# smpurkis/PyTorch-Face-Detection-from-Scratch

Hardware: AMD Instinct MI355X
Metric: train imgs/sec (PoolResnet 480^2, bs=256 per GPU) (higher is better)
Workload: dtype f32 (3x3 convs: bf16x3 split MFMA, fp32 accumulate)

## Files before the change

include/fdet.h:

```cpp
#ifndef FDET_H
#define FDET_H

#include <stddef.h>
#include <stdint.h>

#ifdef __cplusplus
extern "C" {
#endif

#define FDET_VERSION 100
#define FDET_OK 0
#define FDET_EINVAL (-1)
#define FDET_ELAUNCH (-2)
#define FDET_EWORKSPACE (-3)

int fdet_version(void);
const char* fdet_last_error(void);


int fdet_encode_targets(const float* boxes, const int32_t* box_offset, int B, int S,
                        float img_w, float img_h, float* out, void* stream);

int fdet_yolo_loss_fwd_bwd(const float* pred, const float* gt, int B, int S,
                           float* loss_per_image, float* loss_sum, float* grad_pred,
                           float grad_scale, void* stream);

int fdet_decode(const float* maps, int B, int S, float prob_threshold, float img_w, float img_h,
                float* scores, float* boxes, int32_t* counts, void* stream);

int fdet_nms(const float* boxes, const float* scores, const int32_t* counts, int B, int Kmax,
             double iou_threshold, int32_t* keep, int32_t* keep_counts, void* stream);

int fdet_reduce_bounding_boxes(const float* maps, int B, int S, float prob_threshold,
                               double iou_threshold, float img_w, float img_h,
                               float* out, int32_t* out_counts, void* stream);

int fdet_step_metrics(const float* gt, const int32_t* gt_counts, const float* pred,
                      const int32_t* pred_counts, int B, int Kmax, float* per_image,
                      float* totals, void* stream);

// ... 610 lines not shown
```

pytorch-face-detection-from-scratch_amd/_native.py:

```python
from __future__ import annotations

import ctypes
import os
import re
import subprocess
from typing import Optional

import torch

_HERE = os.path.dirname(os.path.abspath(__file__))
LIB_PATH = os.environ.get("FDET_LIB_PATH") or os.path.join(_HERE, "lib", "libfdet_hip.so")
HEADER_PATH = os.path.join(os.path.dirname(_HERE), "include", "fdet.h")


class FdetError(RuntimeError):
    pass


def build(verbose: bool = False) -> str:
    cmd = ["make", "-C", os.path.join(_HERE, "csrc"), "-j", str(min(8, os.cpu_count() or 1))]
    r = subprocess.run(cmd, capture_output=True, text=True)
    if verbose or r.returncode != 0:
        print(r.stdout[-4000:])
        print(r.stderr[-8000:])
    if r.returncode != 0:
        raise FdetError("building libfdet_hip.so failed (see compiler output above)")
    return LIB_PATH


_c = ctypes
_P, _I, _F, _D, _SZ, _U64, _U32 = _c.c_void_p, _c.c_int, _c.c_float, _c.c_double, _c.c_size_t, _c.c_uint64, _c.c_uint32

SIGNATURES = {
    "fdet_version": (_I, []),
    "fdet_last_error": (_c.c_char_p, []),
    "fdet_encode_targets": (_I, [_P, _P, _I, _I, _F, _F, _P, _P]),
    "fdet_yolo_loss_fwd_bwd": (_I, [_P, _P, _I, _I, _P, _P, _P, _F, _P]),
    "fdet_decode": (_I, [_P, _I, _I, _F, _F, _F, _P, _P, _P, _P]),
    "fdet_nms": (_I, [_P, _P, _P, _I, _I, _D, _P, _P, _P]),
    "fdet_reduce_bounding_boxes": (_I, [_P, _I, _I, _F, _D, _F, _F, _P, _P, _P]),
    "fdet_step_metrics": (_I, [_P, _P, _P, _P, _I, _I, _P, _P, _P]),
    "fdet_ssd_num_priors": (_I, [_P, _I]),
    "fdet_ssd_encode_targets": (_I, [_P, _P, _I, _P, _I, _F, _F, _P, _P]),
    "fdet_ssd_loss_ws_bytes": (_SZ, [_I]),
    "fdet_ssd_loss_fwd_bwd": (_I, [_P, _P, _I, _I, _I, _P, _P, _P, _P, _SZ, _P]),
    "fdet_ssd_loss_parts": (_I, [_P, _P, _I, _I, _I, _P, _P, _P, _P, _SZ, _P]),
    "fdet_ssd_loss_finish": (_I, [_P, _P, _P, _SZ, _P, _SZ, _P]),
    "fdet_ssd_reduce_bounding_boxes": (_I, [_P, _I, _P, _I, _I, _F, _D, _F, _F, _P, _P, _P]),
    "fdet_ssd_reduce_bounding_boxes_priors": (_I, [_P, _I, _P, _I, _I, _P, _F, _D, _F, _F, _P, _P, _P]),
    "fdet_ssd_head_pack_fwd": (_I, [_P, _I, _I, _I, _I, _I, _P, _P]),
    "fdet_ssd_head_pack_bwd": (_I, [_P, _P, _I, _I, _I, _I, _I, _P, _P]),
    "fdet_u8_to_f32_norm": (_I, [_P, _P, _SZ, _P]),
    "fdet_resize_bilinear_u8_norm": (_I, [_P, _P, _I, _I, _I, _I, _I, _I, _P]),
    "fdet_resize_bilinear_f32_norm": (_I, [_P, _P, _I, _I, _I, _I, _I, _I, _F, _P]),
    "fdet_adam_step": (_I, [_P, _P, _P, _P, _SZ, _I, _D, _D, _D, _D, _F, _P]),
    "fdet_pack_conv3x3_weights": (_I, [_P, _I, _I, _P, _P, _P]),
    "fdet_conv3x3_fwd": (_I, [_P, _P, _P, _P, _P, _P, _P, _I, _I, _I, _I, _I, _I, _F, _P]),
    "fdet_conv3x3_dgrad": (_I, [_P, _P, _P, _P, _P, _I, _I, _I, _I, _I, _F, _P]),
# ... 221 lines not shown
```

pytorch-face-detection-from-scratch_amd/csrc/fdet_conv3x3_x3.hip:

```cpp
#include "fdet_conv3x3_x3.h"
#include <algorithm>

namespace {

long long* g_probe_stamps = nullptr;
constexpr int PACK_MAXL = 32;
struct PackBatch { const float* w[PACK_MAXL]; bf16x8* fwd[PACK_MAXL]; bf16x8* bwd[PACK_MAXL]; };

__device__ __forceinline__ void pack3x3_x3(const float* __restrict__ w, int Cout, int Cin, int CoP, int CiP,
                                           bf16x8* __restrict__ fwd, bf16x8* __restrict__ bwd) {
  const int nf = (Cin / 16) * 9 * 2 * CoP, nb = (Cout / 16) * 9 * 2 * CiP;
  const int t = blockIdx.x * 256 + threadIdx.x;
  if (fwd && t < nf) {
    const int co = t % CoP, r = t / CoP;
    const int h = r & 1, r2 = r >> 1, tap = r2 % 9, c16 = r2 / 9;
    float f[8];
#pragma unroll
    for (int j = 0; j < 8; ++j) f[j] = (co < Cout) ? w[((size_t)co * Cin + c16 * 16 + 8 * h + j) * 9 + tap] : 0.f;
    bf16x8 hi, lo;
    split8(f, hi, lo);
    fwd[t] = hi;
    fwd[nf + t] = lo;
  }
  if (bwd && t < nb) {
    const int ci = t % CiP, r = t / CiP;
    const int h = r & 1, r2 = r >> 1, tap = r2 % 9, o16 = r2 / 9;
    float f[8];
#pragma unroll
    for (int j = 0; j < 8; ++j) f[j] = (ci < Cin) ? w[((size_t)(o16 * 16 + 8 * h + j) * Cin + ci) * 9 + (8 - tap)] : 0.f;
    bf16x8 hi, lo;
    split8(f, hi, lo);
    bwd[t] = hi;
    bwd[nb + t] = lo;
  }
}

__global__ void __launch_bounds__(256)
k_pack3x3_x3(const float* __restrict__ w, int Cout, int Cin, int CoP, int CiP, bf16x8* __restrict__ fwd,
             bf16x8* __restrict__ bwd) {
  pack3x3_x3(w, Cout, Cin, CoP, CiP, fwd, bwd);
}

__global__ void __launch_bounds__(256)
k_pack3x3_x3_batched(const PackBatch b, int Cout, int Cin, int CoP, int CiP) {
  pack3x3_x3(b.w[blockIdx.y], Cout, Cin, CoP, CiP, b.fwd[blockIdx.y], b.bwd[blockIdx.y]);
}

int run_x3(ConvArgs a, hipStream_t st) {
  static const char kernel_choice = [] { const char* e = getenv("FDET_CONV_KERNEL"); return e ? e[0] : '\0'; }();
  if (a.W <= 64 && kernel_choice != 'g') {
    static const int sb_al = [] { const char* e = getenv("FDET_SB_AL"); return e ? (e[0] == '1' ? 1 : 0) : -1; }();
    if (sb_al == 1 || (sb_al < 0 && a.W >= 33)) {
// ... 284 lines not shown
```

pytorch-face-detection-from-scratch_amd/csrc/fdet_head_fused.hip:

```cpp
#include "fdet_common.h"
#include <cfloat>

using namespace fdet;

typedef __bf16 hf_bf16x8 __attribute__((ext_vector_type(8)));
typedef float hf_f32x4 __attribute__((ext_vector_type(4)));

namespace {

constexpr int HF_T = 512;
constexpr int HF_F = 64;
constexpr int HF_K = 6;
constexpr int HF_KK = HF_K * HF_K;
constexpr int HF_XPT = 248;
constexpr int HF_XTP = 248;
constexpr int HF_DZOFF = (HF_K - 1) * 16 + (HF_K - 1);
constexpr int HF_DZP = 328;
constexpr int HF_DQ = 160;
constexpr int HF_OFF_XB = 0;
constexpr int HF_OFF_XT = HF_OFF_XB + 2 * 8 * HF_XPT * 16;
constexpr int HF_OFF_DZ = HF_OFF_XT + 2 * HF_F * HF_XTP * 2;
constexpr int HF_OFF_DZT = HF_OFF_DZ + 2 * HF_DZP * 16;
constexpr int HF_OFF_PART = HF_OFF_DZT + HF_K * 2 * 5 * HF_DQ * 2;
constexpr int HF_OFF_SC = HF_OFF_PART + 2 * 5 * 160 * 4;
// ... 327 lines not shown
      for (int i = tid; i < a.N; i += 256) s += __hip_atomic_load(a.lpi + i, __ATOMIC_RELAXED, __HIP_MEMORY_SCOPE_AGENT);
      red[tid] = s;
    }
    __syncthreads();
    for (int w = 128; w > 0; w >>= 1) {
      if (tid < w) red[tid] += red[tid + w];
      __syncthreads();
    }
    if (tid == 0) {
      a.lsum[0] = red[0] * 1.0f;
      *a.counter = 0u;
    }
  }
}

__global__ void __launch_bounds__(256)
k_head_fused_pack(const float* __restrict__ w, hf_bf16x8* __restrict__ wf, hf_bf16x8* __restrict__ wd) {
  const int t = blockIdx.x * 256 + threadIdx.x;
  const int nwf = HF_KK * 2 * 4 * 8, nwd = HF_KK * HF_F;
  if (t < nwf) {
    const int slot = t & 7, kgp = (t >> 3) & 3, c32 = (t >> 5) & 1, tap = t >> 6;
    float v[8];
#pragma unroll
    for (int j = 0; j < 8; ++j) v[j] = slot < 5 ? w[((size_t)slot * HF_F + 32 * c32 + 8 * kgp + j) * HF_KK + tap] : 0.f;
    hf_bf16x8 hi, lo;
    hf_split8(v, hi, lo);
    wf[t] = hi;
    wf[nwf + t] = lo;
  } else if (t < nwf + nwd) {
    const int u = t - nwf, c = u & 63, tap = u >> 6;
    float v[8];
#pragma unroll
    for (int j = 0; j < 8; ++j) v[j] = j < 5 ? w[((size_t)j * HF_F + c) * HF_KK + tap] : 0.f;
    hf_bf16x8 hi, lo;
    hf_split8(v, hi, lo);
    wd[u] = hi;
    wd[nwd + u] = lo;
  }
}

__global__ void __launch_bounds__(1024)
k_head_fused_reduce(const float* __restrict__ wsW, const float* __restrict__ wsb, int N, float* __restrict__ dW,
                    float* __restrict__ db) {
  __shared__ float part[1024];
  const int q = threadIdx.x & 63, ph = threadIdx.x >> 6;
  const int nS = HF_KK * 5 * HF_F;
  const int t = blockIdx.x * 64 + q;
  float s = 0.f;
  if (t < nS) {
    for (int n = ph; n < N; n += 16) s += wsW[(size_t)n * nS + t];
  } else if (t < nS + 5) {
    for (int n = ph; n < N; n += 16) s += wsb[(size_t)n * 8 + (t - nS)];
  }
  part[threadIdx.x] = s;
  __syncthreads();
  if (ph == 0) {
    float tot = 0.f;
#pragma unroll
    for (int p = 0; p < 16; ++p) tot += part[p * 64 + q];
    if (t < nS) {
      const int c = t & 63, r = t >> 6, o = r % 5, tap = r / 5;
      dW[((size_t)o * HF_F + c) * HF_KK + tap] = tot;
    } else if (t < nS + 5) {
      db[t - nS] = tot;
    }
  }
}

constexpr size_t hf_pack_units() { return (size_t)2 * HF_KK * 2 * 4 * 8 + (size_t)2 * HF_KK * HF_F; }

}

extern "C" int fdet_head_loss_fused_supported(int F, int H, int W, int k, int pad) {
  const int So = H - k + 1, Wo = W - k + 1;
  return F == HF_F && k == HF_K && pad == 0 && H >= k && W >= k && H <= 15 && W <= 15 && So <= 10 && 5 * So * Wo <= HF_T;
}
// ... 41 lines not shown
```

pytorch-face-detection-from-scratch_amd/csrc/fdet_stem_x3.hip:

```cpp
#include "fdet_common.h"
#include "fdet_ps.h"
#include "fdet_q8_common.h"
#include <algorithm>
#include <cstdlib>
#include <utility>

using namespace fdet;
typedef float f32x16 __attribute__((ext_vector_type(16)));
typedef float f32x4 __attribute__((ext_vector_type(4)));
typedef __bf16 bf16x8 __attribute__((ext_vector_type(8)));
typedef __bf16 bf16x4 __attribute__((ext_vector_type(4)));

namespace {

constexpr int KS = 10, ST = 8, PD = 2, CIN = 3;
constexpr int NROW = CIN * KS;
constexpr int RL = 8 * 64 + 16;
constexpr int RC = RL / 8;
constexpr int NSLOT = 15;

struct StemX3Args {
  const float* x; const float* w; const float* bias; float* y;
  int N, F, H, W, Ho, Wo, nrows;
  int ps_hp, ps_wp, ps_plane, ps_img;
  float q_inv;
};

__global__ void __launch_bounds__(256, 1)
k_stem_fwd_x3(const StemX3Args a) {
  extern __shared__ __attribute__((aligned(16))) char smem[];
  __bf16* Xh = reinterpret_cast<__bf16*>(smem);
  __bf16* Xl = Xh + NROW * RL;
  const int tid = threadIdx.x, lane = tid & 63, wid = tid >> 6;
  const int l31 = lane & 31, half = lane >> 5;
// ... 128 lines not shown
__device__ __forceinline__ unsigned sx_hi_pair(float f0, float f1) {
  typedef __bf16 bf16x2_t __attribute__((ext_vector_type(2)));
  const bf16x2_t h = {(__bf16)f0, (__bf16)f1};
  return __builtin_bit_cast(unsigned, h);
}

template <bool PSO, bool P16 = false, bool U8 = false, bool Q8 = false>
__global__ void __launch_bounds__(256, 1)
k_stem_fwd_x3_pipe(const StemX3Args a) {
  static_assert(PSO || !P16, "precision16 stem: PS output only");
  static_assert(PSO || !U8, "uint8 stem: PS output only");
  static_assert(!Q8 || (PSO && U8 && !P16), "Q8 stem: the uint8-frame bf16x3 form only");
  constexpr int NST = Q8 ? 2 : PSO ? (P16 ? 2 : 4) : 16;
  extern __shared__ __attribute__((aligned(16))) char smem[];
  constexpr int TILE = NROW * RL * 2;
  __bf16* const base = reinterpret_cast<__bf16*>(smem);
  const int tid = threadIdx.x, lane = tid & 63, wid = tid >> 6;
  const int l31 = lane & 31, half = lane >> 5;
  const int m = wid & 1, nt = wid >> 1;
  const int cob = blockIdx.y;
  const int co = cob * 64 + m * 32 + l31;
  const int jmax = a.W / 4;
  float* const sbias = reinterpret_cast<float*>(smem + 2 * TILE * 2);
  {
    f32x4* z = reinterpret_cast<f32x4*>(smem);
    for (int t = tid; t < 2 * TILE * 2 / 16; t += 256) z[t] = f32x4{0.f, 0.f, 0.f, 0.f};
    if (tid < 64) sbias[tid] = cob * 64 + tid < a.F ? a.bias[cob * 64 + tid] : 0.f;
  }
  unsigned* const lut = reinterpret_cast<unsigned*>(smem + 2 * TILE * 2 + 256);
  if (U8) {
    const float f = (float)tid / 255.0f;
    unsigned h_, l_;
    sx_split_pair(f, 0.f, h_, l_);
    lut[tid] = (h_ & 0xffffu) | (l_ << 16);
  }
  bf16x8 ah[NROW], al[NROW];
#pragma unroll
  for (int rr = 0; rr < NROW; ++rr) {
#pragma unroll
    for (int j = 0; j < 8; ++j) {
      const int kx = 8 * half + j - 2;
      const float f = (co < a.F && kx >= 0 && kx < KS) ? a.w[((size_t)co * CIN * KS + rr) * KS + kx] : 0.f;
      const __bf16 h = (__bf16)f;
      ah[rr][j] = h;
      if (!P16) al[rr][j] = (__bf16)(f - (float)h);
    }
  }
  const unsigned long long pa = (unsigned long long)a.x;
  const u32x4s rx = {(unsigned)pa, (unsigned)(pa >> 32), (unsigned)(a.N * CIN * a.H * a.W) * (U8 ? 1u : 4u), 0x00020000u};
  const int j4 = tid & 127, rsub = tid >> 7;
  const bool lane_ok = j4 < jmax;
  f32x4 p0[U8 ? 1 : NSLOT], p1[U8 ? 1 : NSLOT];
  unsigned q0[U8 ? NSLOT : 1], q1[U8 ? NSLOT : 1];
#define SXP_LOAD1(S, SL, RN, ROY)                                                               \
  {                                                                                             \
    const int irow_ = 2 * (SL) + rsub;                                                          \
    const int ci = irow_ / KS, ky = irow_ - ci * KS;                                            \
    const int iy = (ROY) * ST - PD + ky;                                                        \
    const bool ok = lane_ok & ((ROY) >= 0) & (iy >= 0) & (iy < a.H);                           \
    unsigned off = ((unsigned)(((RN) * CIN + ci) * a.H + iy) * a.W + j4 * 4) * (U8 ? 1u : 4u); \
    if constexpr (Q8) {                                                                         \
       \
       \
      off = (unsigned)(((RN) * CIN + ci) * a.H + iy) * a.W;                                     \
      asm volatile("" : "+v"(off));                                                             \
      off += j4 * 4;                                                                            \
    }                                                                                           \
    if constexpr (U8) sx_aload1<S == 0>(q##S[SL], ok ? off : 0x80000000u, rx);                  \
    else sx_aload<S == 0>(p##S[SL], ok ? off : 0x80000000u, rx);                                \
  }
// ... 107 lines not shown
            auto r2 = __builtin_amdgcn_permlane32_swap(la[k], lb[k], false, false);             \
            la[k] = r2[0]; lb[k] = r2[1];                                                       \
          }                                                                                     \
        }                                                                                       \
        const int G = 4 * m + 2 * gp + half;                                                    \
        const unsigned off = (ox < a.Wo && row < last) ? (unsigned)(n * a.ps_img + (G * a.ps_hp + oy) * a.ps_wp + ox + 1) * 16u : 0x80000000u; \
        typedef unsigned sx_u32x4 __attribute__((ext_vector_type(4)));                          \
        __builtin_amdgcn_raw_buffer_store_b128(sx_u32x4{ha[0], ha[1], hb[0], hb[1]}, ry, off, 0, 0); \
        if (!P16) __builtin_amdgcn_raw_buffer_store_b128(sx_u32x4{la[0], la[1], lb[0], lb[1]}, ry, off, a.ps_plane * 16, 0); \
      }                                                                                         \
    } else {                                                                                    \
    _Pragma("unroll") for (int r = 0; r < 16; ++r) {                                            \
      const int c2 = cob * 64 + m * 32 + (r & 3) + 8 * (r >> 2) + 4 * half;                     \
      const bool ok = ox < a.Wo && c2 < a.F && row < last;                                      \
      const unsigned off = ok ? ((unsigned)((n * a.F + c2) * a.Ho + oy) * a.Wo + ox) * 4u : 0x80000000u; \
      __builtin_amdgcn_raw_buffer_store_b32(__builtin_bit_cast(unsigned, acc[r] + sbias[m * 32 + (r & 3) + 8 * (r >> 2) + 4 * half]), ry, off, 0, 0); \
    }                                                                                           \
    }                                                                                           \
    __syncthreads();                                                                            \
    row += 1;                                                                                   \
  }
  const __amdgpu_buffer_rsrc_t ry = __builtin_amdgcn_make_buffer_rsrc(a.y, 0, PSO ? a.N * a.ps_img * 16 : a.N * a.F * a.Ho * a.Wo * 4, 0x00020000);
  const int last2 = row + ((last - row + 1) & ~1);
  while (row < last2) {
    SXP_BAND(0, 1)
    SXP_BAND(1, 0)
  }
  SXP_WAIT(0, 0)
  SXP_WAIT(1, 0)
#undef SXP_BAND
#undef SXP_NOY
#undef SXP_JOB
#undef SXP_WAIT
#undef SXP_LOAD1
}

constexpr int PC = 11;
constexpr int PE = PC * 8;
constexpr int NPLANE = NROW * 8;
constexpr int DL = 72;
constexpr int WSLOT = 4;
typedef __bf16 bf16x2 __attribute__((ext_vector_type(2)));
typedef unsigned u32x4 __attribute__((ext_vector_type(4)));

struct StemWgX3Args {
  const float* x; const float* dy; float* ws; float* wsb;
  int N, F, H, W, Ho, Wo, nrows;
};

__device__ __forceinline__ bf16x8 shift7(const bf16x8& c0, const bf16x8& c1) {
  const u32x4 a = __builtin_bit_cast(u32x4, c0), b = __builtin_bit_cast(u32x4, c1);
  u32x4 o;
// ... 143 lines not shown
  for (int s_ = 0; s_ < 4; ++s_) {
    float v = bpart[s_];
    v += __shfl_xor(v, 8, 16); v += __shfl_xor(v, 4, 16); v += __shfl_xor(v, 2, 16); v += __shfl_xor(v, 1, 16);
    const int c = (s_ * 256 + tid) >> 4;
    if ((tid & 15) == 0) a.wsb[(size_t)blockIdx.x * FP + cob * 64 + c] = v;
  }
}

constexpr int PCP = 9, PEP = PCP * 8;
constexpr int TILEP = NPLANE * PEP * 2;

template <bool P16>
__global__ void __launch_bounds__(256, 1)
k_stem_wgrad_x3_pipe(const StemWgX3Args a) {
  extern __shared__ __attribute__((aligned(16))) char smem[];
  __bf16* const base = reinterpret_cast<__bf16*>(smem);
  __bf16* Dh = base + 2 * TILEP;
  __bf16* Dl = Dh + 64 * DL;
  const int tid = threadIdx.x, lane = tid & 63, wid = tid >> 6;
  const int l31 = lane & 31, half = lane >> 5;
  const int m = wid & 1, ng = wid >> 1;
  const int cob = blockIdx.y;
  const int gmax = a.W / 16, dmax = a.Wo / 4;
  {
    f32x4* z = reinterpret_cast<f32x4*>(smem);
    for (int t = tid; t < (2 * TILEP + 2 * 64 * DL + 8 * PEP) * 2 / 16; t += 256) z[t] = f32x4{0.f, 0.f, 0.f, 0.f};
  }
  int pbase[5];
#pragma unroll
  for (int t = 0; t < 5; ++t) {
    int plane, extra;
    if (t < 4) { const int kk = min((ng * 4 + t) * 32 + l31, NROW * 8 - 1); plane = kk; extra = 1; }
    else { const int kk2 = min(ng * 32 + l31, NROW * 2 - 1); plane = (kk2 >> 1) * 8 + 6 + (kk2 & 1); extra = 0; }
    pbase[t] = plane * PCP + extra + half;
  }
  const bf16x8* Ah = reinterpret_cast<const bf16x8*>(Dh + (m * 32 + l31) * DL) + half;
  const bf16x8* Al = reinterpret_cast<const bf16x8*>(Dl + (m * 32 + l31) * DL) + half;
  f32x16 acc[5];
#pragma unroll
  for (int t = 0; t < 5; ++t)
#pragma unroll
    for (int r = 0; r < 16; ++r) acc[t][r] = 0.f;
  float bpart[4] = {0.f, 0.f, 0.f, 0.f};
  int xw_off[WSLOT]; unsigned x_goff[WSLOT]; bool x_ok[WSLOT];
#pragma unroll
  for (int s_ = 0; s_ < WSLOT; ++s_) {
    const int it = s_ * 256 + tid;
    const int rr = it >> 5, g_ = it & 31;
    x_ok[s_] = rr < NROW && g_ < gmax;
    xw_off[s_] = x_ok[s_] ? (rr * 8) * PEP + 8 + 2 * g_ : -1;
// ... 102 lines not shown
      else { bh = fb[F][0]; if (!P16) bl = fb[F][1]; }                                            \
      if (!P16) {                                                                                 \
        acc[t] = __builtin_amdgcn_mfma_f32_32x32x16_bf16(fa[FA][0], bl, acc[t], 0, 0, 0);         \
        acc[t] = __builtin_amdgcn_mfma_f32_32x32x16_bf16(fa[FA][1], bh, acc[t], 0, 0, 0);         \
      }                                                                                           \
      acc[t] = __builtin_amdgcn_mfma_f32_32x32x16_bf16(fa[FA][0], bh, acc[t], 0, 0, 0);           \
      if constexpr (u + 1 < 20) {                                                                 \
        constexpr int ks1 = (u + 1) / 5, t1 = (u + 1) % 5;                                        \
        if constexpr (t1 == 0) { fa[ks1 & 1][0] = Ah[2 * ks1]; if (!P16) fa[ks1 & 1][1] = Al[2 * ks1]; } \
        fb[F ^ 1][0] = Bh[pbase[t1] + 2 * ks1]; if (!P16) fb[F ^ 1][1] = Bl[pbase[t1] + 2 * ks1]; \
        if constexpr (t1 == 4) { fb[F ^ 1][2] = Bh[pbase[t1] + 2 * ks1 + 1]; if (!P16) fb[F ^ 1][3] = Bl[pbase[t1] + 2 * ks1 + 1]; } \
      }                                                                                           \
      if constexpr (u < 16) { SWP_JOB(0, u / 4, (u % 4) * 2, (PAR) ^ 1) SWP_JOB(0, u / 4, (u % 4) * 2 + 1, (PAR) ^ 1) } \
      if constexpr (u >= 4) SWP_LOAD_X1(0, (u - 4) / 4, (u - 4) % 4, n2_, oy2_)                   \
      __builtin_amdgcn_sched_barrier(0);                                                          \
    });                                                                                           \
    __syncthreads();                                                                              \
    asm volatile("s_waitcnt vmcnt(16)");                                                          \
    SWP_PASS_D()                                                                                  \
    SWP_STAGE_D()                                                                                 \
    __syncthreads();                                                                              \
    row += 1;                                                                                     \
  }
  for (int par = 0; row < last; par ^= 1) SWP_ROW(par)
  asm volatile("s_waitcnt vmcnt(0)");
  SWP_PASS_X(0) SWP_PASS_D()
#undef SWP_ROW
#undef SWP_STAGE_D
#undef SWP_JOB
#undef SWP_PASS_D
#undef SWP_PASS_X
#undef SWP_PASS_XS
#undef SWP_LOAD_D1
#undef SWP_LOAD_X1
#undef SWP_NOY
  const int FP = gridDim.y * 64;
#pragma unroll
  for (int t = 0; t < 5; ++t) {
    const int kp = (t < 4 ? ng * 4 + t : 8 + ng) * 32 + l31;
#pragma unroll
    for (int r = 0; r < 16; ++r) {
      const int c2 = cob * 64 + m * 32 + (r & 3) + 8 * (r >> 2) + 4 * half;
      a.ws[((size_t)blockIdx.x * FP + c2) * 320 + kp] = acc[t][r];
    }
  }
#pragma unroll
  for (int s_ = 0; s_ < 4; ++s_) {
    float v = bpart[s_];
    v += __shfl_xor(v, 8, 16); v += __shfl_xor(v, 4, 16); v += __shfl_xor(v, 2, 16); v += __shfl_xor(v, 1, 16);
    const int c = (s_ * 256 + tid) >> 4;
    if ((tid & 15) == 0) a.wsb[(size_t)blockIdx.x * FP + cob * 64 + c] = v;
  }
}

__global__ void __launch_bounds__(1024)
k_stem_x3_reduce(const float* __restrict__ ws, const float* __restrict__ wsb, int nblk, int F, int FP,
                 float* __restrict__ dW, float* __restrict__ db) {
  __shared__ float part[1024];
  const int f = blockIdx.y;
  const int kq = threadIdx.x & 63, ph = threadIdx.x >> 6;
  const int kp = blockIdx.x * 64 + kq;
  float s = 0.f;
  if (kp < 320)
    for (int b = ph; b < nblk; b += 16) s += ws[((size_t)b * FP + f) * 320 + kp];
  part[threadIdx.x] = s;
  __syncthreads();
  if (ph == 0 && kp < 320) {
    int rr = -1, kx = 0;
    if (kp < 256) { if (kp < NROW * 8) { rr = kp >> 3; kx = (kp & 7) + 2; } }
    else { const int k2 = kp - 256; if (k2 < NROW * 2) { rr = k2 >> 1; kx = k2 & 1; } }
    if (rr >= 0) {
      float tot = 0.f;
#pragma unroll
      for (int p = 0; p < 16; ++p) tot += part[p * 64 + kq];
      dW[((size_t)f * NROW + rr) * KS + kx] = tot;
    }
  }
  __syncthreads();
  if (blockIdx.x == 0) {
    float t = 0.f;
    for (int b = threadIdx.x; b < nblk; b += 1024) t += wsb[(size_t)b * FP + f];
    part[threadIdx.x] = t;
    __syncthreads();
    for (int w = 512; w > 0; w >>= 1) {
      if (threadIdx.x < w) part[threadIdx.x] += part[threadIdx.x + w];
      __syncthreads();
    }
    if (threadIdx.x == 0) db[f] = part[0];
  }
}

}

namespace fdet {

int stem_x3_fwd(const float* x, const float* w, const float* bias, float* y, int N, int F, int H, int W,
                hipStream_t st) {
  StemX3Args a{};
  a.x = x; a.w = w; a.bias = bias; a.y = y; a.N = N; a.F = F; a.H = H; a.W = W;
  a.Ho = (H + 4 - 10) / 8 + 1; a.Wo = (W + 4 - 10) / 8 + 1; a.nrows = N * a.Ho;
  const int FP = (F + 63) / 64 * 64;
  const int nblk = a.nrows < 256 ? a.nrows : 256;
  const size_t lds = (size_t)NROW * RL * 2 * 2;
  const char* e = FDET_ENV_ONCE("FDET_STEM_PIPE");
// ... 150 lines not shown
```

pytorch-face-detection-from-scratch_amd/csrc/fdet_wgrad3x3_ps.hip:

```cpp
#include "fdet_conv3x3_x3.h"
#include "fdet_ps.h"
#include "fdet_ldsdma.h"
#include <algorithm>

using namespace fdet;

typedef __attribute__((address_space(3))) void* lds_void_t;
typedef const __attribute__((address_space(1))) void* glb_void_t;
typedef short s16x4 __attribute__((ext_vector_type(4)));
typedef __attribute__((address_space(3))) s16x4* lds_s16x4_t;
typedef __bf16 bf16x2_t __attribute__((ext_vector_type(2)));
typedef unsigned u32x2_t __attribute__((ext_vector_type(2)));
typedef unsigned u32x4_t __attribute__((ext_vector_type(4)));

namespace {

#ifndef WG_DBG
#define WG_DBG 0
#endif
constexpr int WG_MAXL = 16;
constexpr int XL = 5, ZL = 3;
constexpr int XA = XL * 64 + 4;
constexpr int ZLS = 66;
constexpr int ZA = 212;
constexpr int WG_LDS_UNITS = 16 * XA + 16 * ZA;

struct PsWgArgs {
  const bf16x8* x[WG_MAXL];
  const bf16x8* dz[WG_MAXL];
  float* ws;
  float* wsb;
  int plane, img;
  int lpi, real_lpi, nlines;
  int nslab, lpw;
  unsigned magic_lpi;
};

__device__ __forceinline__ bf16x2_t as_bf16x2(unsigned u) { return __builtin_bit_cast(bf16x2_t, u); }
__device__ __forceinline__ u32x2_t tr2(const char* base, int off) {
  return __builtin_bit_cast(u32x2_t, __builtin_amdgcn_ds_read_tr16_b64_v4i16((lds_s16x4_t)(base + off)));
}
__host__ __device__ constexpr int x_line(int S, int ky, int WP) { return 16 * S + (ky - 1) * WP < 0 ? 0 : (16 * S + (ky - 1) * WP >= 64 ? 2 : 1); }
__host__ __device__ constexpr int x_off(int S, int ky, int WP) {
  return 16 * S + (ky - 1) * WP < 0 ? 16 * S + (ky - 1) * WP + 64 : (16 * S + (ky - 1) * WP >= 64 ? 16 * S + (ky - 1) * WP - 64 : 16 * S + (ky - 1) * WP);
}

template <int WP, bool P16 = false>
__global__ void __launch_bounds__(256, 1)
k_wgrad3x3_ps(const PsWgArgs a) {
  extern __shared__ __attribute__((aligned(16))) char smem[];
  bf16x8* const lds = reinterpret_cast<bf16x8*>(smem);
  const int tid = threadIdx.x, lane = tid & 63;
  const int wid = __builtin_amdgcn_readfirstlane(tid >> 6);
  const int m = wid & 1, j = wid >> 1;
  const int layer = blockIdx.y;
  const bf16x8* __restrict__ gx = a.x[layer];
  const bf16x8* __restrict__ gz = a.dz[layer];
  {
    f32x4* z = reinterpret_cast<f32x4*>(smem);
    for (int t = tid; t < WG_LDS_UNITS; t += 256) z[t] = f32x4{0.f, 0.f, 0.f, 0.f};
  }
  const int i16 = lane & 15, g16 = (lane >> 4) & 1, kh = lane >> 5;
  const int q = i16 >> 2, pp = i16 & 3;
  const int GA = 4 * m + 2 * g16 + (pp >> 1), GB = 4 * j + 2 * g16 + (pp >> 1);
  const int lane_x = (GB * XA + 8 * kh + q) * 16 + (pp & 1) * 8;
  const int lane_z = (16 * XA + GA * ZA + 1 + 8 * kh + q) * 16 + (pp & 1) * 8;
  constexpr int XPL = 8 * XA * 16, ZPL = 8 * ZA * 16;

  const int l0 = blockIdx.x * a.lpw, l1 = min(l0 + a.lpw, a.nlines);
  f32x16 acc[9];
#pragma unroll
  for (int t = 0; t < 9; ++t)
#pragma unroll
    for (int r = 0; r < 16; ++r) acc[t][r] = 0.f;
  float bsum = 0.f;
  const unsigned bsel0 = j == 0 ? 0x3f803f80u : 0u, bsel1 = j == 1 ? 0x3f803f80u : 0u;

  const unsigned lds0 = (unsigned)(size_t)(lds_void_t)smem;
  const unsigned tbytes = (unsigned)((a.nlines / a.lpi) + 2) * (unsigned)a.img * 16u;
  const dma_u32x4 xrs = dma_rsrc(gx - a.img, tbytes), zrs = dma_rsrc(gz - a.img, tbytes);
  const unsigned lane16 = (unsigned)lane * 16u;
#define WG_PIECE(RS, LG, AI, DST)                                                                  \
  {                                                                                                \
    const int lg_ = (LG) + a.lpi;                                                                  \
    const int n_ = (int)__umulhi((unsigned)lg_, a.magic_lpi);                                      \
    const unsigned so_ = (unsigned)(n_ * a.img + ((AI) >> 3) * a.plane + ((AI) & 7) * (a.lpi * 64) + (lg_ - n_ * a.lpi) * 64) * 16u; \
    dma_piece(lds0 + (unsigned)(DST) * 16u, lane16, RS, so_);                                      \
  }
#define WG_ISSUE(LX, SX, LZ, SZ)                                                                   \
  if (!(P16 && wid >= 2)) {                                   \
    _Pragma("unroll") for (int k_ = 0; k_ < 4; ++k_) {                                             \
      const int ai_ = 4 * wid + k_;                                                                \
      WG_PIECE(xrs, LX, ai_, ai_ * XA + (SX) * 64)                                                  \
      WG_PIECE(zrs, LZ, ai_, 16 * XA + ai_ * ZA + (SZ) * ZLS + 1)                                   \
    }                                                                                              \
  }
  __syncthreads();
  int sx = ((l0 - 1) % XL + XL) % XL, sz = l0 % ZL;
#define XS(D) ((sx + (D)) % XL)
  WG_ISSUE(l0 - 1, XS(0), l0, sz)
  WG_ISSUE(l0, XS(1), l0 + 1, (sz + 1) % ZL)
  if (!(P16 && wid >= 2)) {
    _Pragma("unroll") for (int k_ = 0; k_ < 4; ++k_) {
      const int ai_ = 4 * wid + k_;
      WG_PIECE(xrs, l0 + 1, ai_, ai_ * XA + XS(2) * 64)
      WG_PIECE(xrs, l0 + 2, ai_, ai_ * XA + XS(3) * 64)
    }
  }
  asm volatile("s_waitcnt vmcnt(0)" ::: "memory");

  u32x4_t zf[2][3][2], xf[2][3][2];
#define WG_FRAGS(F, S, ZB, XB0, XB1, XB2)                                                          \
  {                                                                                                \
    _Pragma("unroll") for (int k_ = 0; k_ < 3; ++k_)                                               \
      _Pragma("unroll") for (int pl_ = 0; pl_ < (P16 ? 1 : 2); ++pl_)                              \
        _Pragma("unroll") for (int h_ = 0; h_ < 2; ++h_) {                                         \
          const u32x2_t z_ = (WG_DBG & 4) ? u32x2_t{0x3f803f80u + (unsigned)lane, 0x40004000u} : tr2(ZB, pl_ * ZPL + (16 * (S) + 4 * h_ - (k_ - 1)) * 16); \
          zf[F][k_][pl_][2 * h_] = z_[0]; zf[F][k_][pl_][2 * h_ + 1] = z_[1];                      \
          const char* xb_ = x_line((S), k_, WP) == 0 ? XB0 : (x_line((S), k_, WP) == 1 ? XB1 : XB2); \
          const u32x2_t x_ = (WG_DBG & 4) ? u32x2_t{0x3f803f80u, 0x40004000u + (unsigned)lane} : tr2(xb_, pl_ * XPL + (x_off((S), k_, WP) + 4 * h_) * 16); \
          xf[F][k_][pl_][2 * h_] = x_[0]; xf[F][k_][pl_][2 * h_ + 1] = x_[1];                      \
        }                                                                                          \
  }
  int band = l0;
  {
    __builtin_amdgcn_s_barrier();
    const char* zb_ = smem + lane_z + sz * (ZLS * 16);
    const char* xb0 = smem + lane_x + XS(0) * 1024;
    const char* xb1 = smem + lane_x + XS(1) * 1024;
    const char* xb2 = smem + lane_x + XS(2) * 1024;
    WG_FRAGS(0, 0, zb_, xb0, xb1, xb2)
  }
  int row = l0 - (l0 / a.lpi) * a.lpi;
  while (band < l1) {
  const int n_full = row < a.real_lpi ? min(l1 - band, a.real_lpi - row) : 0;
  row += n_full;
  for (const int bend = band + n_full; band < bend; ++band) {
    asm volatile("s_waitcnt vmcnt(0)" ::: "memory");
    __builtin_amdgcn_s_barrier();
    if (!(WG_DBG & 1)) WG_ISSUE(band + 3, XS(4), band + 2, (sz + 2) % ZL)
    __builtin_amdgcn_sched_barrier(0);
    {
      const char* zb_ = smem + lane_z + sz * (ZLS * 16);
      const char* xb0 = smem + lane_x + XS(0) * 1024;
      const char* xb1 = smem + lane_x + XS(1) * 1024;
      const char* xb2 = smem + lane_x + XS(2) * 1024;
      const char* zbn = smem + lane_z + ((sz + 1) % ZL) * (ZLS * 16);
      const char* xb3 = smem + lane_x + XS(3) * 1024;
#pragma unroll
      for (int s = 0; s < 4; ++s) {
        const int F = s & 1;
        if (s < 3) WG_FRAGS(F ^ 1, s + 1, zb_, xb0, xb1, xb2)
        else WG_FRAGS(0, 0, zbn, xb1, xb2, xb3)
#pragma unroll
        for (int ky = 0; ky < 3; ++ky)
// ... 41 lines not shown
    sz = (sz + 1) % ZL;
  }
  if (band < l1 && row >= a.real_lpi) {
    const int n_zero = min(l1 - band, a.lpi - row);
    for (const int bend = band + n_zero; band < bend; ++band) {
      asm volatile("s_waitcnt vmcnt(0)" ::: "memory");
      __builtin_amdgcn_s_barrier();
      if (!(WG_DBG & 1)) WG_ISSUE(band + 3, XS(4), band + 2, (sz + 2) % ZL)
      sx = (sx + 1) % XL;
      sz = (sz + 1) % ZL;
    }
    row += n_zero;
    if (row >= a.lpi) row = 0;
    if (band < l1) {
      const char* zb_ = smem + lane_z + sz * (ZLS * 16);
      const char* xb0 = smem + lane_x + XS(0) * 1024;
      const char* xb1 = smem + lane_x + XS(1) * 1024;
      const char* xb2 = smem + lane_x + XS(2) * 1024;
      WG_FRAGS(0, 0, zb_, xb0, xb1, xb2)
    }
  }
  }
  asm volatile("s_waitcnt vmcnt(0)" ::: "memory");
#undef WG_FRAGS
#undef XS
#undef WG_ISSUE
#undef WG_PIECE
  const int l31 = lane & 31, half = lane >> 5;
  const size_t s = (size_t)layer * a.nslab + blockIdx.x;
  float* __restrict__ wsl = a.ws + s * 9 * 64 * 64;
#pragma unroll
  for (int t = 0; t < 9; ++t)
#pragma unroll
    for (int r = 0; r < 16; ++r) {
      const int co = 32 * m + (r & 3) + 8 * (r >> 2) + 4 * half;
      wsl[(t * 64 + co) * 64 + 32 * j + l31] = acc[t][r];
    }
  bsum += __shfl_xor(bsum, 32, 64);
  if (half == 0) a.wsb[(s * 2 + j) * 64 + 32 * m + l31] = bsum;
}

struct PsWgRed { float* dW[WG_MAXL]; float* db[WG_MAXL]; };
__global__ void __launch_bounds__(256)
k_wgrad_ps_reduce(const float* __restrict__ ws, const float* __restrict__ wsb, int nslab, const PsWgRed out) {
  __shared__ float part[256];
  const int layer = blockIdx.y;
  const int el = threadIdx.x & 63, q = threadIdx.x >> 6;
  const bool bias_blk = blockIdx.x == 9 * 64;
  const size_t stride = bias_blk ? 128 : 9 * 4096;
  const float* __restrict__ src = bias_blk ? wsb + (size_t)layer * nslab * 128 + el
                                           : ws + (size_t)layer * nslab * 9 * 4096 + (size_t)blockIdx.x * 64 + el;
  float s = 0.f;
  int k = q;
  for (; k + 28 < nslab; k += 32) {
    float v[8];
#pragma unroll
    for (int u = 0; u < 8; ++u) v[u] = src[(size_t)(k + 4 * u) * stride] + (bias_blk ? src[(size_t)(k + 4 * u) * stride + 64] : 0.f);
#pragma unroll
    for (int u = 0; u < 8; ++u) s += v[u];
  }
  for (; k < nslab; k += 4) s += src[(size_t)k * stride] + (bias_blk ? src[(size_t)k * stride + 64] : 0.f);
  part[threadIdx.x] = s;
  __syncthreads();
  if (q == 0) {
    const float r = ((part[el] + part[64 + el]) + part[128 + el]) + part[192 + el];
    if (bias_blk) {
      out.db[layer][el] = r;
    } else {
      const int e = blockIdx.x * 64 + el;
      const int t = e >> 12, co = (e >> 6) & 63, ci = e & 63;
      out.dW[layer][(co * 64 + ci) * 9 + t] = r;
    }
  }
}

int wg_plan(int L, int N, int H, int W, PsGeo& g, int& nslab, int& lpw) {
  PsStrips sp;
  if (!ps_geo_strips(N, 64, H, W, g, sp) || L < 1 || L > WG_MAXL) return 0;
  const int lpi = g.HP * g.WP / 64;
  const long nlines = (long)g.N * lpi;
  if (nlines + 2 * lpi >= (1 << 20) || (size_t)(g.N + 2) * g.img * 16 >= ((size_t)1 << 32)) return 0;
  nslab = std::max(1, std::min((int)nlines, num_cus() / L));
  lpw = (int)((nlines + nslab - 1) / nslab);
  nslab = (int)((nlines + lpw - 1) / lpw);
// ... 28 lines not shown
    red.db[l] = h_db[l];
  }
  a.ws = reinterpret_cast<float*>(ws);
  a.wsb = a.ws + (size_t)L * nslab * 9 * 4096;
  a.plane = g.plane; a.img = g.img;
  a.lpi = g.HP * g.WP / 64;
  a.real_lpi = (H * g.WP + 63) / 64;
  a.nlines = g.N * a.lpi;
  a.nslab = nslab; a.lpw = lpw;
  a.magic_lpi = magic_of(a.lpi);
  const size_t lds = (size_t)WG_LDS_UNITS * 16;
  hipStream_t st = (hipStream_t)stream;
  auto go = [&](auto kern, bool& done) -> int {
    if (!done) {
      if (hipFuncSetAttribute((const void*)kern, hipFuncAttributeMaxDynamicSharedMemorySize, (int)lds) != hipSuccess) {
        (void)hipGetLastError();
        return fail(FDET_ELAUNCH, "conv3x3_wgrad_ps: cannot reserve %zu bytes of LDS", lds);
      }
      done = true;
    }
    hipLaunchKernelGGL(kern, dim3(nslab, L), dim3(256), lds, st, a);
    return FDET_OK;
  };
  static bool d64 = false, d32 = false, d16 = false, d64p = false, d32p = false, d16p = false;
  int rc0;
  if (p16) {
    if (g.WP == 64) rc0 = go(k_wgrad3x3_ps<64, true>, d64p);
    else if (g.WP == 16) rc0 = go(k_wgrad3x3_ps<16, true>, d16p);
    else rc0 = go(k_wgrad3x3_ps<32, true>, d32p);
  }
  else if (g.WP == 64) rc0 = go(k_wgrad3x3_ps<64>, d64);
  else if (g.WP == 16) rc0 = go(k_wgrad3x3_ps<16>, d16);
  else rc0 = go(k_wgrad3x3_ps<32>, d32);
  if (rc0 != FDET_OK) return rc0;
  int rc = check_launch("fdet_conv3x3_wgrad_ps_batched");
  if (rc != FDET_OK) return rc;
  hipLaunchKernelGGL(k_wgrad_ps_reduce, dim3(9 * 64 + 1, L), dim3(256), 0, st, a.ws, a.wsb, nslab, red);
  return check_launch("fdet_conv3x3_wgrad_ps_batched(reduce)");
}
}

extern "C" int fdet_conv3x3_wgrad_ps_batched(const void* const* h_x, const void* const* h_dz, float* const* h_dW,
                                             float* const* h_db, int L, int N, int C, int H, int W, void* ws,
                                             size_t ws_bytes, void* stream) {
  return wgrad_ps_run(h_x, h_dz, h_dW, h_db, L, N, C, H, W, ws, ws_bytes, stream, false);
}

extern "C" int fdet_conv3x3_wgrad_ps_batched_p16(const void* const* h_x, const void* const* h_dz, float* const* h_dW,
                                                 float* const* h_db, int L, int N, int C, int H, int W, void* ws,
                                                 size_t ws_bytes, void* stream) {
  return wgrad_ps_run(h_x, h_dz, h_dW, h_db, L, N, C, H, W, ws, ws_bytes, stream, true);
}
```

Before: 92580.

## Unroll slab reductions, specialize wgrad for one-line images, add debug and stamp hooks

Adds a shared slab_sum helper that issues many independent clamped loads before accumulating. The wgrad, stem and head partial-sum reductions use it to get more memory-level parallelism, and the wgrad reduce unroll factor is chosen from the slab count. Adds an LPI1 template specialization of the wgrad kernel that skips the magic-number division when lpi is 1. Weight packing now loads unconditionally from clamped indices and masks afterwards. Also adds compile-time-gated timestamp probes and a debug LDS-fill entry point, which cost nothing unless enabled.

```diff
diff --git a/include/fdet.h b/include/fdet.h
--- a/include/fdet.h
+++ b/include/fdet.h
@@ -16,6 +16,7 @@
 
 int fdet_version(void);
 const char* fdet_last_error(void);
+int fdet_debug_lds_fill(unsigned pattern, void* stream);
 
 
 int fdet_encode_targets(const float* boxes, const int32_t* box_offset, int B, int S,
diff --git a/pytorch-face-detection-from-scratch_amd/_native.py b/pytorch-face-detection-from-scratch_amd/_native.py
--- a/pytorch-face-detection-from-scratch_amd/_native.py
+++ b/pytorch-face-detection-from-scratch_amd/_native.py
@@ -34,6 +34,7 @@
 SIGNATURES = {
     "fdet_version": (_I, []),
     "fdet_last_error": (_c.c_char_p, []),
+    "fdet_debug_lds_fill": (_I, [_U32, _P]),
     "fdet_encode_targets": (_I, [_P, _P, _I, _I, _F, _F, _P, _P]),
     "fdet_yolo_loss_fwd_bwd": (_I, [_P, _P, _I, _I, _P, _P, _P, _F, _P]),
     "fdet_decode": (_I, [_P, _I, _I, _F, _F, _F, _P, _P, _P, _P]),
diff --git a/pytorch-face-detection-from-scratch_amd/csrc/fdet_conv3x3_x3.hip b/pytorch-face-detection-from-scratch_amd/csrc/fdet_conv3x3_x3.hip
--- a/pytorch-face-detection-from-scratch_amd/csrc/fdet_conv3x3_x3.hip
+++ b/pytorch-face-detection-from-scratch_amd/csrc/fdet_conv3x3_x3.hip
@@ -16,7 +16,9 @@
     const int h = r & 1, r2 = r >> 1, tap = r2 % 9, c16 = r2 / 9;
     float f[8];
 #pragma unroll
-    for (int j = 0; j < 8; ++j) f[j] = (co < Cout) ? w[((size_t)co * Cin + c16 * 16 + 8 * h + j) * 9 + tap] : 0.f;
+    for (int j = 0; j < 8; ++j) f[j] = w[((size_t)min(co, Cout - 1) * Cin + c16 * 16 + 8 * h + j) * 9 + tap];
+#pragma unroll
+    for (int j = 0; j < 8; ++j) f[j] = (co < Cout) ? f[j] : 0.f;
     bf16x8 hi, lo;
     split8(f, hi, lo);
     fwd[t] = hi;
@@ -27,7 +29,9 @@
     const int h = r & 1, r2 = r >> 1, tap = r2 % 9, o16 = r2 / 9;
     float f[8];
 #pragma unroll
-    for (int j = 0; j < 8; ++j) f[j] = (ci < Cin) ? w[((size_t)(o16 * 16 + 8 * h + j) * Cin + ci) * 9 + (8 - tap)] : 0.f;
+    for (int j = 0; j < 8; ++j) f[j] = w[((size_t)(o16 * 16 + 8 * h + j) * Cin + min(ci, Cin - 1)) * 9 + (8 - tap)];
+#pragma unroll
+    for (int j = 0; j < 8; ++j) f[j] = (ci < Cin) ? f[j] : 0.f;
     bf16x8 hi, lo;
     split8(f, hi, lo);
     bwd[t] = hi;
diff --git a/pytorch-face-detection-from-scratch_amd/csrc/fdet_debug.hip b/pytorch-face-detection-from-scratch_amd/csrc/fdet_debug.hip
--- /dev/null
+++ b/pytorch-face-detection-from-scratch_amd/csrc/fdet_debug.hip
@@ -0,0 +1,27 @@
+#include "fdet_common.h"
+
+using namespace fdet;
+
+namespace {
+
+__global__ void __launch_bounds__(256)
+k_debug_lds_fill(unsigned pattern, int nwords) {
+  extern __shared__ __attribute__((aligned(16))) unsigned dbg_lds[];
+  volatile unsigned* l = dbg_lds;
+  for (int i = threadIdx.x; i < nwords; i += 256) l[i] = pattern;
+}
+
+}
+
+extern "C" int fdet_debug_lds_fill(unsigned pattern, void* stream) {
+  int dev = 0, lds = 0;
+  if (hipGetDevice(&dev) != hipSuccess ||
+      hipDeviceGetAttribute(&lds, hipDeviceAttributeMaxSharedMemoryPerBlock, dev) != hipSuccess || lds < 4) {
+    (void)hipGetLastError();
+    return fail(FDET_ELAUNCH, "debug_lds_fill: cannot query the LDS size");
+  }
+  lds &= ~15;
+  if (int rc = set_lds_attr((const void*)k_debug_lds_fill, (size_t)lds, "debug_lds_fill")) return rc;
+  hipLaunchKernelGGL(k_debug_lds_fill, dim3(4 * num_cus()), dim3(256), lds, (hipStream_t)stream, pattern, lds / 4);
+  return check_launch("fdet_debug_lds_fill");
+}
diff --git a/pytorch-face-detection-from-scratch_amd/csrc/fdet_head_fused.hip b/pytorch-face-detection-from-scratch_amd/csrc/fdet_head_fused.hip
--- a/pytorch-face-detection-from-scratch_amd/csrc/fdet_head_fused.hip
+++ b/pytorch-face-detection-from-scratch_amd/csrc/fdet_head_fused.hip
@@ -1,4 +1,5 @@
 #include "fdet_common.h"
+#include "fdet_slabsum.h"
 #include <cfloat>
 
 using namespace fdet;
@@ -373,7 +374,9 @@
     const int slot = t & 7, kgp = (t >> 3) & 3, c32 = (t >> 5) & 1, tap = t >> 6;
     float v[8];
 #pragma unroll
-    for (int j = 0; j < 8; ++j) v[j] = slot < 5 ? w[((size_t)slot * HF_F + 32 * c32 + 8 * kgp + j) * HF_KK + tap] : 0.f;
+    for (int j = 0; j < 8; ++j) v[j] = w[((size_t)min(slot, 4) * HF_F + 32 * c32 + 8 * kgp + j) * HF_KK + tap];
+#pragma unroll
+    for (int j = 0; j < 8; ++j) v[j] = slot < 5 ? v[j] : 0.f;
     hf_bf16x8 hi, lo;
     hf_split8(v, hi, lo);
     wf[t] = hi;
@@ -398,11 +401,8 @@
   const int nS = HF_KK * 5 * HF_F;
   const int t = blockIdx.x * 64 + q;
   float s = 0.f;
-  if (t < nS) {
-    for (int n = ph; n < N; n += 16) s += wsW[(size_t)n * nS + t];
-  } else if (t < nS + 5) {
-    for (int n = ph; n < N; n += 16) s += wsb[(size_t)n * 8 + (t - nS)];
-  }
+  if (t < nS) s = slab_sum<16>(wsW + t, nS, ph, 16, N);
+  else if (t < nS + 5) s = slab_sum<16>(wsb + (t - nS), 8, ph, 16, N);
   part[threadIdx.x] = s;
   __syncthreads();
   if (ph == 0) {
diff --git a/pytorch-face-detection-from-scratch_amd/csrc/fdet_slabsum.h b/pytorch-face-detection-from-scratch_amd/csrc/fdet_slabsum.h
--- /dev/null
+++ b/pytorch-face-detection-from-scratch_amd/csrc/fdet_slabsum.h
@@ -0,0 +1,25 @@
+#pragma once
+#include <hip/hip_runtime.h>
+
+namespace fdet {
+
+template <int U, bool PAIR = false>
+__device__ __forceinline__ float slab_sum(const float* __restrict__ p, size_t stride, int k0, int step, int n,
+                                          int pair_off = 0) {
+  float s = 0.f;
+  for (int k = k0; k < n; k += U * step) {
+    float v[U], w[PAIR ? U : 1];
+#pragma unroll
+    for (int u = 0; u < U; ++u) {
+      const float* __restrict__ e = p + (size_t)min(k + u * step, n - 1) * stride;
+      v[u] = e[0];
+      if (PAIR) w[u] = e[pair_off];
+    }
+#pragma unroll
+    for (int u = 0; u < U; ++u)
+      if (k + u * step < n) s += PAIR ? v[u] + w[u] : v[u];
+  }
+  return s;
+}
+
+}
diff --git a/pytorch-face-detection-from-scratch_amd/csrc/fdet_stamps.h b/pytorch-face-detection-from-scratch_amd/csrc/fdet_stamps.h
--- /dev/null
+++ b/pytorch-face-detection-from-scratch_amd/csrc/fdet_stamps.h
@@ -0,0 +1,22 @@
+#pragma once
+#ifdef FDET_TAIL_STAMPS
+#include <hip/hip_runtime.h>
+#define FDET_STAMP_MAXWG 4096
+#define FDET_STAMP_DECL(TU)                                                                        \
+  __device__ long long* g_stamps_##TU = nullptr;                                                   \
+  extern "C" int fdet_stamps_set_##TU(long long* buf) {                                            \
+    return hipMemcpyToSymbol(HIP_SYMBOL(g_stamps_##TU), &buf, sizeof(buf)) == hipSuccess ? 0 : -3; \
+  }
+#define FDET_STAMP(TU, KID, I)                                                                     \
+  {                                                                                                \
+    __builtin_amdgcn_sched_barrier(0);                                                             \
+    const unsigned wg_ = blockIdx.y * gridDim.x + blockIdx.x;                                      \
+    if (g_stamps_##TU && threadIdx.x == 0 && wg_ < FDET_STAMP_MAXWG)                               \
+      g_stamps_##TU[((size_t)(KID) * FDET_STAMP_MAXWG + wg_) * 8 + (I)] =                          \
+          ((I) == 4 || (I) == 5) ? (long long)__builtin_amdgcn_s_memrealtime() : (long long)__builtin_amdgcn_s_memtime(); \
+    __builtin_amdgcn_sched_barrier(0);                                                             \
+  }
+#else
+#define FDET_STAMP_DECL(TU)
+#define FDET_STAMP(TU, KID, I)
+#endif
diff --git a/pytorch-face-detection-from-scratch_amd/csrc/fdet_stem_x3.hip b/pytorch-face-detection-from-scratch_amd/csrc/fdet_stem_x3.hip
--- a/pytorch-face-detection-from-scratch_amd/csrc/fdet_stem_x3.hip
+++ b/pytorch-face-detection-from-scratch_amd/csrc/fdet_stem_x3.hip
@@ -1,6 +1,8 @@
 #include "fdet_common.h"
 #include "fdet_ps.h"
 #include "fdet_q8_common.h"
+#include "fdet_slabsum.h"
+#include "fdet_stamps.h"
 #include <algorithm>
 #include <cstdlib>
 #include <utility>
@@ -10,6 +12,8 @@
 typedef float f32x4 __attribute__((ext_vector_type(4)));
 typedef __bf16 bf16x8 __attribute__((ext_vector_type(8)));
 typedef __bf16 bf16x4 __attribute__((ext_vector_type(4)));
+
+FDET_STAMP_DECL(stem)
 
 namespace {
 
@@ -184,11 +188,13 @@
   const int co = cob * 64 + m * 32 + l31;
   const int jmax = a.W / 4;
   float* const sbias = reinterpret_cast<float*>(smem + 2 * TILE * 2);
+  FDET_STAMP(stem, 1, 0) FDET_STAMP(stem, 1, 4)
   {
     f32x4* z = reinterpret_cast<f32x4*>(smem);
     for (int t = tid; t < 2 * TILE * 2 / 16; t += 256) z[t] = f32x4{0.f, 0.f, 0.f, 0.f};
     if (tid < 64) sbias[tid] = cob * 64 + tid < a.F ? a.bias[cob * 64 + tid] : 0.f;
   }
+  FDET_STAMP(stem, 1, 7)
   unsigned* const lut = reinterpret_cast<unsigned*>(smem + 2 * TILE * 2 + 256);
   if (U8) {
     const float f = (float)tid / 255.0f;
@@ -208,6 +214,10 @@
       if (!P16) al[rr][j] = (__bf16)(f - (float)h);
     }
   }
+#ifdef FDET_TAIL_STAMPS
+  asm volatile("s_waitcnt vmcnt(0)" ::: "memory");
+#endif
+  FDET_STAMP(stem, 1, 6)
   const unsigned long long pa = (unsigned long long)a.x;
   const u32x4s rx = {(unsigned)pa, (unsigned)(pa >> 32), (unsigned)(a.N * CIN * a.H * a.W) * (U8 ? 1u : 4u), 0x00020000u};
   const int j4 = tid & 127, rsub = tid >> 7;
@@ -361,12 +371,14 @@
   }
   const __amdgpu_buffer_rsrc_t ry = __builtin_amdgcn_make_buffer_rsrc(a.y, 0, PSO ? a.N * a.ps_img * 16 : a.N * a.F * a.Ho * a.Wo * 4, 0x00020000);
   const int last2 = row + ((last - row + 1) & ~1);
+  FDET_STAMP(stem, 1, 1)
   while (row < last2) {
     SXP_BAND(0, 1)
     SXP_BAND(1, 0)
   }
   SXP_WAIT(0, 0)
   SXP_WAIT(1, 0)
+  FDET_STAMP(stem, 1, 2) FDET_STAMP(stem, 1, 3) FDET_STAMP(stem, 1, 5)
 #undef SXP_BAND
 #undef SXP_NOY
 #undef SXP_JOB
@@ -556,10 +568,12 @@
   const int m = wid & 1, ng = wid >> 1;
   const int cob = blockIdx.y;
   const int gmax = a.W / 16, dmax = a.Wo / 4;
+  FDET_STAMP(stem, 2, 0) FDET_STAMP(stem, 2, 4)
   {
     f32x4* z = reinterpret_cast<f32x4*>(smem);
     for (int t = tid; t < (2 * TILEP + 2 * 64 * DL + 8 * PEP) * 2 / 16; t += 256) z[t] = f32x4{0.f, 0.f, 0.f, 0.f};
   }
+  FDET_STAMP(stem, 2, 7)
   int pbase[5];
 #pragma unroll
   for (int t = 0; t < 5; ++t) {
@@ -708,9 +722,11 @@
     __syncthreads();                                                                              \
     row += 1;                                                                                     \
   }
+  FDET_STAMP(stem, 2, 1)
   for (int par = 0; row < last; par ^= 1) SWP_ROW(par)
   asm volatile("s_waitcnt vmcnt(0)");
   SWP_PASS_X(0) SWP_PASS_D()
+  FDET_STAMP(stem, 2, 2)
 #undef SWP_ROW
 #undef SWP_STAGE_D
 #undef SWP_JOB
@@ -737,6 +753,11 @@
     const int c = (s_ * 256 + tid) >> 4;
     if ((tid & 15) == 0) a.wsb[(size_t)blockIdx.x * FP + cob * 64 + c] = v;
   }
+#ifdef FDET_TAIL_STAMPS
+  asm volatile("s_waitcnt vmcnt(0)" ::: "memory");
+  __syncthreads();
+#endif
+  FDET_STAMP(stem, 2, 3) FDET_STAMP(stem, 2, 5)
 }
 
 __global__ void __launch_bounds__(1024)
@@ -746,9 +767,11 @@
   const int f = blockIdx.y;
   const int kq = threadIdx.x & 63, ph = threadIdx.x >> 6;
   const int kp = blockIdx.x * 64 + kq;
+  float t = 0.f;
+  if (blockIdx.x == 0)
+    for (int b = threadIdx.x; b < nblk; b += 1024) t += wsb[(size_t)b * FP + f];
   float s = 0.f;
-  if (kp < 320)
-    for (int b = ph; b < nblk; b += 16) s += ws[((size_t)b * FP + f) * 320 + kp];
+  if (kp < 320) s = slab_sum<16>(ws + (size_t)f * 320 + kp, (size_t)FP * 320, ph, 16, nblk);
   part[threadIdx.x] = s;
   __syncthreads();
   if (ph == 0 && kp < 320) {
@@ -764,8 +787,6 @@
   }
   __syncthreads();
   if (blockIdx.x == 0) {
-    float t = 0.f;
-    for (int b = threadIdx.x; b < nblk; b += 1024) t += wsb[(size_t)b * FP + f];
     part[threadIdx.x] = t;
     __syncthreads();
     for (int w = 512; w > 0; w >>= 1) {
diff --git a/pytorch-face-detection-from-scratch_amd/csrc/fdet_wgrad3x3_ps.hip b/pytorch-face-detection-from-scratch_amd/csrc/fdet_wgrad3x3_ps.hip
--- a/pytorch-face-detection-from-scratch_amd/csrc/fdet_wgrad3x3_ps.hip
+++ b/pytorch-face-detection-from-scratch_amd/csrc/fdet_wgrad3x3_ps.hip
@@ -1,6 +1,8 @@
 #include "fdet_conv3x3_x3.h"
 #include "fdet_ps.h"
 #include "fdet_ldsdma.h"
+#include "fdet_slabsum.h"
+#include "fdet_stamps.h"
 #include <algorithm>
 
 using namespace fdet;
@@ -12,6 +14,8 @@
 typedef __bf16 bf16x2_t __attribute__((ext_vector_type(2)));
 typedef unsigned u32x2_t __attribute__((ext_vector_type(2)));
 typedef unsigned u32x4_t __attribute__((ext_vector_type(4)));
+
+FDET_STAMP_DECL(wgps)
 
 namespace {
 
@@ -45,7 +49,7 @@
   return 16 * S + (ky - 1) * WP < 0 ? 16 * S + (ky - 1) * WP + 64 : (16 * S + (ky - 1) * WP >= 64 ? 16 * S + (ky - 1) * WP - 64 : 16 * S + (ky - 1) * WP);
 }
 
-template <int WP, bool P16 = false>
+template <int WP, bool P16 = false, bool LPI1 = false>
 __global__ void __launch_bounds__(256, 1)
 k_wgrad3x3_ps(const PsWgArgs a) {
   extern __shared__ __attribute__((aligned(16))) char smem[];
@@ -56,6 +60,7 @@
   const int layer = blockIdx.y;
   const bf16x8* __restrict__ gx = a.x[layer];
   const bf16x8* __restrict__ gz = a.dz[layer];
+  FDET_STAMP(wgps, (WP == 64 ? 0 : WP == 32 ? 1 : 2),0) FDET_STAMP(wgps, (WP == 64 ? 0 : WP == 32 ? 1 : 2),4)
   {
     f32x4* z = reinterpret_cast<f32x4*>(smem);
     for (int t = tid; t < WG_LDS_UNITS; t += 256) z[t] = f32x4{0.f, 0.f, 0.f, 0.f};
@@ -83,7 +88,7 @@
 #define WG_PIECE(RS, LG, AI, DST)                                                                  \
   {                                                                                                \
     const int lg_ = (LG) + a.lpi;                                                                  \
-    const int n_ = (int)__umulhi((unsigned)lg_, a.magic_lpi);                                      \
+    const int n_ = LPI1 ? lg_ : (int)__umulhi((unsigned)lg_, a.magic_lpi);                         \
     const unsigned so_ = (unsigned)(n_ * a.img + ((AI) >> 3) * a.plane + ((AI) & 7) * (a.lpi * 64) + (lg_ - n_ * a.lpi) * 64) * 16u; \
     dma_piece(lds0 + (unsigned)(DST) * 16u, lane16, RS, so_);                                      \
   }
@@ -96,6 +101,7 @@
     }                                                                                              \
   }
   __syncthreads();
+  FDET_STAMP(wgps, (WP == 64 ? 0 : WP == 32 ? 1 : 2),6)
   int sx = ((l0 - 1) % XL + XL) % XL, sz = l0 % ZL;
 #define XS(D) ((sx + (D)) % XL)
   WG_ISSUE(l0 - 1, XS(0), l0, sz)
@@ -131,6 +137,7 @@
     const char* xb2 = smem + lane_x + XS(2) * 1024;
     WG_FRAGS(0, 0, zb_, xb0, xb1, xb2)
   }
+  FDET_STAMP(wgps, (WP == 64 ? 0 : WP == 32 ? 1 : 2),1)
   int row = l0 - (l0 / a.lpi) * a.lpi;
   while (band < l1) {
   const int n_full = row < a.real_lpi ? min(l1 - band, a.real_lpi - row) : 0;
@@ -218,6 +225,7 @@
   }
   }
   asm volatile("s_waitcnt vmcnt(0)" ::: "memory");
+  FDET_STAMP(wgps, (WP == 64 ? 0 : WP == 32 ? 1 : 2),2)
 #undef WG_FRAGS
 #undef XS
 #undef WG_ISSUE
@@ -234,28 +242,24 @@
     }
   bsum += __shfl_xor(bsum, 32, 64);
   if (half == 0) a.wsb[(s * 2 + j) * 64 + 32 * m + l31] = bsum;
+#ifdef FDET_TAIL_STAMPS
+  asm volatile("s_waitcnt vmcnt(0)" ::: "memory");
+  __syncthreads();
+#endif
+  FDET_STAMP(wgps, (WP == 64 ? 0 : WP == 32 ? 1 : 2),3) FDET_STAMP(wgps, (WP == 64 ? 0 : WP == 32 ? 1 : 2),5)
 }
 
 struct PsWgRed { float* dW[WG_MAXL]; float* db[WG_MAXL]; };
+template <int U>
 __global__ void __launch_bounds__(256)
 k_wgrad_ps_reduce(const float* __restrict__ ws, const float* __restrict__ wsb, int nslab, const PsWgRed out) {
   __shared__ float part[256];
   const int layer = blockIdx.y;
   const int el = threadIdx.x & 63, q = threadIdx.x >> 6;
   const bool bias_blk = blockIdx.x == 9 * 64;
-  const size_t stride = bias_blk ? 128 : 9 * 4096;
-  const float* __restrict__ src = bias_blk ? wsb + (size_t)layer * nslab * 128 + el
-                                           : ws + (size_t)layer * nslab * 9 * 4096 + (size_t)blockIdx.x * 64 + el;
-  float s = 0.f;
-  int k = q;
-  for (; k + 28 < nslab; k += 32) {
-    float v[8];
-#pragma unroll
-    for (int u = 0; u < 8; ++u) v[u] = src[(size_t)(k + 4 * u) * stride] + (bias_blk ? src[(size_t)(k + 4 * u) * stride + 64] : 0.f);
-#pragma unroll
-    for (int u = 0; u < 8; ++u) s += v[u];
-  }
-  for (; k < nslab; k += 4) s += src[(size_t)k * stride] + (bias_blk ? src[(size_t)k * stride + 64] : 0.f);
+  float s;
+  if (bias_blk) s = slab_sum<U, true>(wsb + (size_t)layer * nslab * 128 + el, 128, q, 4, nslab, 64);
+  else s = slab_sum<U>(ws + (size_t)layer * nslab * 9 * 4096 + (size_t)blockIdx.x * 64 + el, 9 * 4096, q, 4, nslab);
   part[threadIdx.x] = s;
   __syncthreads();
   if (q == 0) {
@@ -330,9 +334,10 @@
     hipLaunchKernelGGL(kern, dim3(nslab, L), dim3(256), lds, st, a);
     return FDET_OK;
   };
-  static bool d64 = false, d32 = false, d16 = false, d64p = false, d32p = false, d16p = false;
+  static bool d64 = false, d32 = false, d16 = false, d64p = false, d32p = false, d16p = false, d16l = false, d16pl = false;
   int rc0;
-  if (p16) {
+  if (a.lpi == 1) rc0 = p16 ? go(k_wgrad3x3_ps<16, true, true>, d16pl) : go(k_wgrad3x3_ps<16, false, true>, d16l);
+  else if (p16) {
     if (g.WP == 64) rc0 = go(k_wgrad3x3_ps<64, true>, d64p);
     else if (g.WP == 16) rc0 = go(k_wgrad3x3_ps<16, true>, d16p);
     else rc0 = go(k_wgrad3x3_ps<32, true>, d32p);
@@ -343,7 +348,12 @@
   if (rc0 != FDET_OK) return rc0;
   int rc = check_launch("fdet_conv3x3_wgrad_ps_batched");
   if (rc != FDET_OK) return rc;
-  hipLaunchKernelGGL(k_wgrad_ps_reduce, dim3(9 * 64 + 1, L), dim3(256), 0, st, a.ws, a.wsb, nslab, red);
+  const int per = (nslab + 3) / 4;
+  auto reduce = [&](auto kern) { hipLaunchKernelGGL(kern, dim3(9 * 64 + 1, L), dim3(256), 0, st, a.ws, a.wsb, nslab, red); };
+  if (per <= 4) reduce(k_wgrad_ps_reduce<4>);
+  else if (per <= 16) reduce(k_wgrad_ps_reduce<16>);
+  else if (per <= 32) reduce(k_wgrad_ps_reduce<32>);
+  else reduce(k_wgrad_ps_reduce<64>);
   return check_launch("fdet_conv3x3_wgrad_ps_batched(reduce)");
 }
 }
```

After: 92790 (median of 6 runs). Within noise of the previous version (+0.2%).
